# synnada-ai/datafusion-upstream

Measured on AMD Instinct MI355X. Metric: rows/sec hash-join+agg, TPC-H SF100 Q3, higher is better.
Workload: dtype int64; 1 GPU; TPC-H SF100 Q3 (3-way hash join + group-by SUM + sort), int64 keys, Decimal128(15,2) money, resident in HBM; input_rows=765043119, parallelism=1 GPU

## Files before the change

datafusion-upstream_amd/csrc/core.hip:

```cpp
#include "device_utils.h"
#include <mutex>

namespace dfgpu {

void fail(dfgpu_status code, const char* fmt, ...) {
  char buf[1024]; va_list ap; va_start(ap, fmt); vsnprintf(buf, sizeof buf, fmt, ap); va_end(ap);
  throw Error(code, buf);
}

struct CtxRefs { std::atomic<int64_t> n{1}; };
static std::mutex g_mu;
static std::vector<std::pair<dfgpu_ctx*, CtxRefs*>> g_ctx;
static CtxRefs* refs_of(dfgpu_ctx* c) { std::lock_guard<std::mutex> l(g_mu); for (auto& p : g_ctx) if (p.first == c) return p.second; return nullptr; }
static void ctx_unref(dfgpu_ctx* c) {
  CtxRefs* r = refs_of(c);
  if (!r || r->n.fetch_sub(1) != 1) return;
  { std::lock_guard<std::mutex> l(g_mu); for (size_t i = 0; i < g_ctx.size(); i++) if (g_ctx[i].first == c) { g_ctx.erase(g_ctx.begin() + i); break; } }
  (void)hipSetDevice(c->device);
  (void)hipStreamSynchronize(c->stream);
  if (c->free_blocks) { for (auto& b : *c->free_blocks) (void)hipFree(b.second); delete c->free_blocks; }
  delete c->alloc_mu;
  if (c->d_flags) (void)hipFree(c->d_flags);
  if (c->d_scratch64) (void)hipFree(c->d_scratch64);
  if (c->h_pinned) (void)hipHostFree(c->h_pinned);
// ... 294 lines not shown
  const int64_t c = counts[i];
  if (c < 0 || c > (int64_t)(0x7FFFFFF0u / w)) { atomicOr(flags, DFGPU_FLAG_OOB); lens[i] = 0; } else lens[i] = (uint32_t)c * w;
}
__global__ void __launch_bounds__(BLOCK) k_list_row_of(const int32_t* offsets, int64_t n, int64_t ne, uint32_t w, uint32_t* row_of) {
  const int64_t e = (int64_t)blockIdx.x * BLOCK + threadIdx.x; if (e >= ne) return;
  const int64_t at = (int64_t)offsets[0] + e * w;
  int64_t lo = 0, hi = n - 1;
  while (lo < hi) { const int64_t mid = (lo + hi + 1) >> 1; if ((int64_t)offsets[mid] <= at) lo = mid; else hi = mid - 1; }
  row_of[e] = (uint32_t)lo;
}
__global__ void __launch_bounds__(BLOCK) k_slist_sizes(const int32_t* voff, int64_t nv, uint32_t* enc) {
  const int64_t j = (int64_t)blockIdx.x * BLOCK + threadIdx.x; if (j > nv) return;
  enc[j] = j == nv ? 0u : 4u + (uint32_t)(voff[j + 1] - voff[j]);
}
__global__ void __launch_bounds__(BLOCK) k_slist_offsets(const uint32_t* cpre , const uint32_t* epos , int64_t n, int32_t* out_off) {
  const int64_t i = (int64_t)blockIdx.x * BLOCK + threadIdx.x; if (i <= n) out_off[i] = (int32_t)epos[cpre[i]];
}
__global__ void __launch_bounds__(BLOCK) k_slist_encode(const int32_t* voff, const uint8_t* vbytes, int64_t nv, const uint32_t* epos, uint8_t* out) {
  const int64_t j = (int64_t)blockIdx.x * BLOCK + threadIdx.x; if (j >= nv) return;
  const uint32_t len = (uint32_t)(voff[j + 1] - voff[j]); uint8_t* o = out + epos[j]; const uint8_t* src = vbytes + voff[j];
  o[0] = (uint8_t)len; o[1] = (uint8_t)(len >> 8); o[2] = (uint8_t)(len >> 16); o[3] = (uint8_t)(len >> 24);
  for (uint32_t b = 0; b < len; b++) o[4 + b] = src[b];
}
__global__ void __launch_bounds__(BLOCK) k_slist_walk(const int32_t* loff, const uint8_t* lbytes, int64_t n, const uint32_t* vstart, uint32_t* cnt, uint32_t* lens, uint32_t* spos, uint32_t* row_of, uint32_t* flags) {
  const int64_t i = (int64_t)blockIdx.x * BLOCK + threadIdx.x; if (i >= n) return;
  int64_t at = loff[i]; const int64_t end = loff[i + 1]; uint32_t k = 0;
  while (at < end) {
    if (at + 4 > end) { atomicOr(flags, DFGPU_FLAG_OOB); break; }
    const uint32_t len = (uint32_t)lbytes[at] | ((uint32_t)lbytes[at + 1] << 8) | ((uint32_t)lbytes[at + 2] << 16) | ((uint32_t)lbytes[at + 3] << 24);
    if (at + 4 + (int64_t)len > end) { atomicOr(flags, DFGPU_FLAG_OOB); break; }
    if (lens) { const uint32_t v = vstart[i] + k; lens[v] = len; spos[v] = (uint32_t)(at + 4); row_of[v] = (uint32_t)i; }
    k++; at += 4 + (int64_t)len;
  }
  if (cnt) cnt[i] = k;
}
__global__ void __launch_bounds__(BLOCK) k_slist_copy(const uint8_t* lbytes, const uint32_t* spos, const int32_t* voff, int64_t nv, uint8_t* out) {
  const int64_t j = (int64_t)blockIdx.x * BLOCK + threadIdx.x; if (j >= nv) return;
  const uint32_t len = (uint32_t)(voff[j + 1] - voff[j]); const uint8_t* src = lbytes + spos[j]; uint8_t* o = out + voff[j];
  for (uint32_t b = 0; b < len; b++) o[b] = src[b];
}

struct CtxOption { const char* name; int64_t (*get)(const dfgpu_ctx*); void (*set)(dfgpu_ctx*, int64_t); };
#define OPT_GET(M) [](const dfgpu_ctx* c) -> int64_t { return (int64_t)c->M; }
#define OPT_BOOL(M) OPT_GET(M), [](dfgpu_ctx* c, int64_t v) { c->M = v != 0; }
#define OPT_INT(M) OPT_GET(M), [](dfgpu_ctx* c, int64_t v) { c->M = v; }
#define OPT_MIN(M, LO) OPT_GET(M), [](dfgpu_ctx* c, int64_t v) { c->M = v < LO ? LO : v; }
#define OPT_RANGE(M, LO, HI) OPT_GET(M), [](dfgpu_ctx* c, int64_t v) { if (v < LO || v > HI) fail(DFGPU_INVALID_ARGUMENT, #M ": " #LO " .. " #HI); c->M = v; }
#define OPT_READ(M) OPT_GET(M), nullptr
static const CtxOption kCtxOptions[] = {
  { "force_hash_collisions", OPT_BOOL(force_hash_collisions) },
  { "first_seen_group_order", OPT_BOOL(first_seen_group_order) },
  { "join_rank_index", OPT_BOOL(join_rank_index) },
  { "join_rank_index_unsorted", OPT_BOOL(join_rank_index_unsorted) },
  { "join_lazy_build_rows", OPT_BOOL(join_lazy_build_rows) },
  { "join_selection_output", OPT_BOOL(join_selection_output) },
  { "join_probe_fused_filter", OPT_BOOL(join_probe_fused_filter) },
  { "join_key_packing", OPT_BOOL(join_key_packing) },
  { "join_swap_small_semi", OPT_BOOL(join_swap_small_semi) },
  { "join_partitioned", OPT_BOOL(join_partitioned) },
  { "join_partitioned_min_build", OPT_INT(join_partitioned_min_build) },
  { "join_partitioned_min_probe", OPT_INT(join_partitioned_min_probe) },
  { "join_partitioned_big", OPT_BOOL(join_partitioned_big) },
  { "join_partitioned_hashed", OPT_BOOL(join_partitioned_hashed) },
  { "join_partitioned_hash_mask", [](const dfgpu_ctx* c) -> int64_t { return c->join_partitioned_hash_mask == ~0ull ? 0 : (int64_t)c->join_partitioned_hash_mask; },
                                  [](dfgpu_ctx* c, int64_t v) { c->join_partitioned_hash_mask = v <= 0 ? ~0ull : (uint64_t)v; } },
  { "join_partition_rows", OPT_INT(join_partition_rows) },
  { "group_run_detection", OPT_BOOL(group_run_detection) },
  { "group_lazy_keys", OPT_BOOL(group_lazy_keys) },
  { "group_dictionary_canon", OPT_BOOL(group_dictionary_canon) },
  { "fused_aggregate_min_rows", OPT_INT(fused_aggregate_min_rows) },
  { "agg_order_inverse_map", OPT_BOOL(agg_order_inverse_map) },
  { "agg_partitioned", OPT_BOOL(agg_partitioned) },
  { "agg_partitioned_force", OPT_BOOL(agg_partitioned_force) },
  { "agg_partitioned_min_rows", OPT_INT(agg_partitioned_min_rows) },
  { "agg_pack_estimate_min_rows", OPT_INT(agg_pack_estimate_min_rows) },
  { "agg_preaggregate_distinct", OPT_READ(pa_last_distinct) },
  { "agg_spill_state_bytes", OPT_INT(agg_spill_state_bytes) },
  { "agg_spill_ranges", OPT_RANGE(agg_spill_ranges, 1, 4096) },
  { "sort_packed_keys", OPT_BOOL(sort_packed_keys) },
  { "sort_packed_min_rows", OPT_MIN(sort_packed_min_rows, 2) },
  { "sort_estimate_ranges", OPT_BOOL(sort_estimate_ranges) },
  { "sort_topk_words_min_rows", OPT_MIN(sort_topk_words_min_rows, 2) },
  { "sort_one_block_max_rows", OPT_MIN(sort_one_block_max_rows, 0) },
  { "sort_onesweep_min_rows", OPT_MIN(sort_onesweep_min_rows, 2) },
  { "sort_onesweep_rows", OPT_GET(sort_onesweep_rows), [](dfgpu_ctx* c, int64_t v) { c->sort_onesweep_rows = v == 16 ? 16 : v > 0 ? 8 : 0; } },
  { "sort_onesweep_fused_finish", OPT_BOOL(sort_onesweep_fused_finish) },
  { "sort_fused_small_passes", OPT_BOOL(sort_fused_small_passes) },
  { "sort_spill_bytes", OPT_INT(sort_spill_bytes) },
  { "sort_spill_ranges", OPT_RANGE(sort_spill_ranges, 1, 4096) },
  { "spm_merge_rows", OPT_GET(spm_merge_rows), [](dfgpu_ctx* c, int64_t v) { if (v < 0) fail(DFGPU_INVALID_ARGUMENT, "spm_merge_rows: >= 0"); c->spm_merge_rows = v; } },
  { "memory_limit", OPT_INT(memory_limit) },
  { "live_bytes", OPT_READ(live_bytes) },
  { "cached_bytes", OPT_READ(cached_bytes) },
  { "trim_cache", nullptr, [](dfgpu_ctx* c, int64_t) {
      HIP_CHECK(hipStreamSynchronize(c->stream));
      std::lock_guard<std::mutex> l(*c->alloc_mu); for (auto& x : *c->free_blocks) (void)hipFree(x.second); c->free_blocks->clear(); c->cached_bytes = 0; } },
  { "mailbox_readback", OPT_BOOL(mailbox_readback) },
  { "collect_metrics", OPT_BOOL(collect_metrics) },
  { "defer_flag_checks", OPT_GET(defer_flag_checks), [](dfgpu_ctx* c, int64_t v) {
      if (v) c->defer_flag_checks++;
      else { if (c->defer_flag_checks > 0) c->defer_flag_checks--; if (c->defer_flag_checks == 0) flush_flags(c); } } },
};
#undef OPT_GET
#undef OPT_BOOL
#undef OPT_INT
#undef OPT_MIN
// ... 406 lines not shown
```

datafusion-upstream_amd/csrc/dfgpu_internal.h:

```cpp
#pragma once
#include <hip/hip_runtime.h>
#include <atomic>
#include <cstdarg>
#include <cstdint>
#include <cstdio>
#include <cstring>
#include <memory>
#include <mutex>
#include <stdexcept>
#include <string>
#include <vector>
#include "../../include/dfgpu.h"

namespace dfgpu {

struct Error : std::exception {
  dfgpu_status code; std::string msg;
  Error(dfgpu_status c, std::string m) : code(c), msg(std::move(m)) {}
  const char* what() const noexcept override { return msg.c_str(); }
};
[[noreturn]] void fail(dfgpu_status code, const char* fmt, ...);

#define HIP_CHECK(expr)                                                                         \
  do { hipError_t e_ = (expr);                                                                  \
    if (e_ != hipSuccess) ::dfgpu::fail(e_ == hipErrorOutOfMemory ? DFGPU_RESOURCES_EXHAUSTED : DFGPU_INTERNAL, \
                                        "%s failed: %s (%s:%d)", #expr, hipGetErrorString(e_), __FILE__, __LINE__); } while (0)
#define KERNEL_CHECK() HIP_CHECK(hipGetLastError())

}

enum : uint32_t { DFGPU_FLAG_DIV_ZERO = 1, DFGPU_FLAG_OVERFLOW = 2, DFGPU_FLAG_CAST = 4, DFGPU_FLAG_OOB = 8, DFGPU_FLAG_TABLE_FULL = 16, DFGPU_FLAG_STALLED = 32 };

namespace dfgpu { struct Buffer; }
struct dfgpu_ctx {
  int device = 0;
  hipStream_t stream = nullptr;
  bool own_stream = false;
  hipStream_t copy_stream = nullptr;
  std::string err;
  bool force_hash_collisions = false;
  bool first_seen_group_order = true;
  bool join_rank_index = true;
  bool join_lazy_build_rows = true;
  bool join_selection_output = true;
  bool join_probe_fused_filter = true;
  bool join_rank_index_unsorted = true;
  bool join_key_packing = true;
  bool group_run_detection = true;
  bool group_lazy_keys = true;
  bool group_dictionary_canon = true;
  bool join_swap_small_semi = true;
  uint64_t join_partitioned_hash_mask = ~0ull;
  bool join_partitioned_hashed = true;
  bool join_partitioned_big = true;
  bool join_partitioned = true; int64_t join_partitioned_min_build = 1 << 20, join_partitioned_min_probe = 1 << 22, join_partition_rows = 14000;
  int64_t fused_aggregate_min_rows = 1 << 20;
  bool sort_packed_keys = true;
  bool agg_partitioned = true, agg_partitioned_force = false; int64_t agg_partitioned_min_rows = 1 << 22;
  bool agg_order_inverse_map = true;
  int64_t agg_pack_estimate_min_rows = 1 << 22;
  bool pa_last_distinct = false;
  const void* pa_sample_key = nullptr; const void* pa_sample_mask = nullptr; int64_t pa_sample_n = 0; uint64_t pa_sample[3] = {0, 0, 0};
  std::shared_ptr<dfgpu::Buffer> pa_pack; int pa_pack_n = 0; int64_t pa_pack_min[4] = {0, 0, 0, 0}; uint64_t pa_pack_stride[4] = {0, 0, 0, 0}, pa_pack_range[4] = {0, 0, 0, 0}; bool pa_pack_nullable[4] = {false, false, false, false};
  std::shared_ptr<dfgpu::Buffer> row_selection; int64_t row_selection_len = 0;
  int defer_flag_checks = 0; bool flags_pending = false; std::string flags_what;
  uint32_t* d_flags = nullptr;
  uint64_t* d_scratch64 = nullptr;
  uint64_t* h_pinned = nullptr;
  static constexpr int MAIL_SEQ = 384, MAIL_WORDS = 256, PINNED_WORDS = 512;
  bool mailbox_readback = true; uint64_t mail_seq = 0;
  int num_cus = 256;
  std::mutex* alloc_mu = nullptr;
  std::vector<std::pair<size_t, void*>>* free_blocks = nullptr;
  size_t cached_bytes = 0, live_bytes = 0;
  int64_t sort_packed_min_rows = 1 << 20;
  int64_t sort_topk_words_min_rows = 1 << 23;
  int64_t sort_one_block_max_rows = 8192;
  int64_t sort_onesweep_min_rows = 1 << 20;
  bool sort_onesweep_fused_finish = true;
  int sort_onesweep_rows = 16;
  bool sort_fused_small_passes = true;
  bool sort_estimate_ranges = true;
  int64_t spm_merge_rows = (int64_t)1 << 25;
  int64_t sort_spill_bytes = 0, sort_spill_ranges = 16;
  int64_t agg_spill_state_bytes = 0, agg_spill_ranges = 16;
  int64_t memory_limit = 0;
  bool collect_metrics = false;
  struct Span { hipEvent_t start = nullptr, stop = nullptr; };
  std::vector<Span> spans;
  std::mutex span_mu;
  bool profile = false; std::string profile_only;
  std::vector<std::pair<std::string, int64_t>> sync_counts;
  void count_sync(const char* why) { if (!profile) return; for (auto& kv : sync_counts) if (kv.first == why) { kv.second++; return; } sync_counts.emplace_back(why, 1); }
  struct ProfRec { const char* name; hipEvent_t start, stop; };
  std::vector<ProfRec> prof;
};

namespace dfgpu {

// ... 143 lines not shown
```

datafusion-upstream_amd/csrc/join.hip:

```cpp
#include "join_table.h"

namespace dfgpu {
constexpr uint64_t SLOT_EMPTY = ~0ull;
constexpr uint32_t NO_SLOT = 0xFFFFFFFFu;
}
using namespace dfgpu;


namespace dfgpu {

__device__ inline bool row_selected(const uint64_t* mask, int64_t i) { return mask == nullptr || bit_get(mask, i); }

__global__ void __launch_bounds__(BLOCK) k_join_build(KeySet ks, int64_t n, const uint64_t* mask, int null_eq, int force_zero,
                                                      uint64_t* slots, uint32_t* slot_count, uint64_t cap_mask, uint32_t* row_slot,
                                                      unsigned long long* counters ) {
  int64_t i = (int64_t)blockIdx.x * BLOCK + threadIdx.x;
  if (i >= n) return;
  uint32_t my_slot = NO_SLOT;
  if (row_selected(mask, i)) {
    bool any_null; uint64_t h = keyset_hash(ks, i, 0, &any_null);
    if (force_zero) h = 0;
    if (!any_null || null_eq) {
      uint64_t tag = h >> 32, s = h & cap_mask, mine = (tag << 32) | (uint64_t)i;
      for (uint64_t step = 0; step <= cap_mask; step++) {
// ... 231 lines not shown
__global__ void __launch_bounds__(BLOCK) k_key_setbits(const T* keys, const uint32_t* row_slot, int64_t n, int64_t kmin, uint64_t* bitmap) {
  int64_t i = (int64_t)blockIdx.x * BLOCK + threadIdx.x;
  if (i >= n || row_slot[i] == NO_SLOT) return;
  uint64_t d = (uint64_t)((int64_t)keys[i] - kmin);
  atomicOr((unsigned long long*)&bitmap[d >> 6], 1ull << (d & 63));
}
template <typename T>
__global__ void __launch_bounds__(BLOCK) k_check_increasing(const T* keys, int64_t n, unsigned long long* out ) {
  bool bad = false, dup = false;
  for (int64_t i = (int64_t)blockIdx.x * BLOCK + threadIdx.x + 1; i < n; i += (int64_t)gridDim.x * BLOCK) { T a = keys[i - 1], b = keys[i]; bad |= b < a; dup |= a == b; }
  if (ballot64(bad) && lane_id() == 0) out[0] = 1ull;
  if (ballot64(dup) && lane_id() == 0) out[3] = 1ull;
  if (blockIdx.x == 0 && threadIdx.x == 0) { out[1] = (unsigned long long)(long long)keys[0]; out[2] = (unsigned long long)(long long)keys[n - 1]; }
}
template <typename T>
__global__ void __launch_bounds__(BLOCK) k_key_setbits_unique(const T* keys, const uint64_t* mask, const uint32_t* rows, const unsigned long long* d_count, int64_t n, int64_t kmin, uint64_t* bitmap, unsigned long long* dup, const T* ckeys = nullptr) {
  const int64_t m = rows ? (int64_t)*d_count : n;
  for (int64_t j = (int64_t)blockIdx.x * BLOCK + threadIdx.x; j < m; j += (int64_t)gridDim.x * BLOCK) {
    const int64_t i = rows ? (int64_t)rows[j] : j;
    if (!rows && mask && !bit_get(mask, i)) continue;
    const uint64_t d = (uint64_t)((int64_t)(ckeys ? ckeys[j] : keys[i]) - kmin), bit = 1ull << (d & 63);
    const unsigned long long old = atomicOr((unsigned long long*)&bitmap[d >> 6], (unsigned long long)bit);
    if (old & bit) *dup = 1ull;
  }
}
template <typename T>
__global__ void __launch_bounds__(BLOCK) k_rank_rows(const T* keys, const uint64_t* mask, const uint32_t* rows, const unsigned long long* d_count, int64_t n, int64_t kmin, const uint64_t* bitmap, const uint32_t* prefix, uint32_t* row_of_rank, const T* ckeys = nullptr) {
  const int64_t m = rows ? (int64_t)*d_count : n;
  for (int64_t j = (int64_t)blockIdx.x * BLOCK + threadIdx.x; j < m; j += (int64_t)gridDim.x * BLOCK) {
    const int64_t i = rows ? (int64_t)rows[j] : j;
    if (!rows && mask && !bit_get(mask, i)) continue;
    const uint64_t d = (uint64_t)((int64_t)(ckeys ? ckeys[j] : keys[i]) - kmin);
    row_of_rank[prefix[d >> 6] + (uint32_t)__popcll(bitmap[d >> 6] & ((1ull << (d & 63)) - 1ull))] = (uint32_t)i;
  }
}
template <typename T>
__global__ void __launch_bounds__(BLOCK) k_key_run_heads(const T* keys, int64_t n, uint64_t* heads) {
  int64_t i = (int64_t)blockIdx.x * BLOCK + threadIdx.x;
  bool h = i < n && (i == 0 || keys[i - 1] != keys[i]);
  uint64_t m = ballot64(h);
  if (lane_id() == 0 && (i >> 6) < ((n + 63) >> 6)) heads[i >> 6] = m;
}
template <typename T>
__global__ void __launch_bounds__(BLOCK) k_probe_lookup_runs(const T* pkeys, const uint32_t* rows, int64_t m, int64_t kmin, const uint64_t* bitmap, const uint32_t* prefix,
                                                             const uint32_t* run_starts, int64_t n_runs, int64_t n_build, uint32_t* out_run, uint32_t* out_cnt) {
  int64_t i = (int64_t)blockIdx.x * BLOCK + threadIdx.x;
  if (i >= m) return;
  uint64_t d = (uint64_t)((int64_t)pkeys[rows[i]] - kmin);
  uint32_t r = prefix[d >> 6] + (uint32_t)__popcll(bitmap[d >> 6] & ((1ull << (d & 63)) - 1ull));
  uint32_t st = run_starts[r], en = (int64_t)r + 1 < n_runs ? run_starts[r + 1] : (uint32_t)n_build;
  out_run[i] = r; out_cnt[i] = en - st;
}
template <typename T>
__global__ void __launch_bounds__(BLOCK) k_key_setbits_masked(const T* keys, const uint64_t* mask, int64_t n, int64_t kmin, uint64_t* bitmap) {
  int64_t i = (int64_t)blockIdx.x * BLOCK + threadIdx.x;
  int lane = lane_id();
  bool on = i < n && row_selected(mask, i);
  uint64_t d = on ? (uint64_t)((int64_t)keys[i] - kmin) : 0;
  int64_t w = on ? (int64_t)(d >> 6) : -1 - lane;
  uint64_t b = on ? 1ull << (d & 63) : 0ull;
#pragma unroll
  for (int s = 1; s < WAVE; s <<= 1) {
    uint64_t ob = __shfl_up(b, s, 64); int64_t ow = __shfl_up(w, s, 64);
    if (lane >= s && ow == w) b |= ob;
  }
  int64_t nxt = __shfl_down(w, 1, 64);
  if (on && (lane == WAVE - 1 || nxt != w)) atomicOr((unsigned long long*)&bitmap[w], (unsigned long long)b);
}
template <typename T>
__global__ void __launch_bounds__(BLOCK) k_key_setbits_rows(const T* keys, const uint32_t* rows, const unsigned long long* d_count, int64_t kmin, uint64_t* bitmap) {
  const int64_t m = (int64_t)*d_count; const int lane = lane_id();
  for (int64_t j0 = (int64_t)blockIdx.x * BLOCK; j0 < m; j0 += (int64_t)gridDim.x * BLOCK) {
    const int64_t j = j0 + threadIdx.x; const bool on = j < m;
    uint64_t d = on ? (uint64_t)((int64_t)keys[rows[j]] - kmin) : 0;
    int64_t w = on ? (int64_t)(d >> 6) : -1 - lane;
    uint64_t b = on ? 1ull << (d & 63) : 0ull;
#pragma unroll
    for (int s2 = 1; s2 < WAVE; s2 <<= 1) {
      uint64_t ob = __shfl_up(b, s2, 64); int64_t ow = __shfl_up(w, s2, 64);
      if (lane >= s2 && ow == w) b |= ob;
    }
    int64_t nxt = __shfl_down(w, 1, 64);
    if (on && (lane == WAVE - 1 || nxt != w)) atomicOr((unsigned long long*)&bitmap[w], (unsigned long long)b);
  }
}
__global__ void __launch_bounds__(BLOCK) k_popc_words(const uint64_t* words, int64_t nw, uint32_t* out) {
  int64_t i = (int64_t)blockIdx.x * BLOCK + threadIdx.x;
  if (i < nw) out[i] = (uint32_t)__popcll(words[i]);
}
constexpr int LR_ROWS = 4;
template <typename T, bool ALL, bool SEL>
__global__ void __launch_bounds__(BLOCK) k_probe_lookup_rank(const T* pkeys, const uint32_t* rows, int64_t m, int64_t kmin, const uint64_t* bitmap,
                                                             const uint32_t* prefix, const uint32_t* sel_rows, int identity, uint64_t* out_build,
                                                             const uint64_t* rows_valid = nullptr, int64_t n_probe = 0) {
  const int64_t base = (int64_t)blockIdx.x * BLOCK * LR_ROWS + threadIdx.x;
  int64_t ic[LR_ROWS]; uint64_t d[LR_ROWS], r[LR_ROWS];
#pragma unroll
  for (int q = 0; q < LR_ROWS; q++) { int64_t i = base + (int64_t)q * BLOCK; ic[q] = i < m ? i : m - 1; }
  bool live[LR_ROWS];
#pragma unroll
  for (int q = 0; q < LR_ROWS; q++) live[q] = rows_valid == nullptr || valid_at(rows_valid, ic[q]);
  if constexpr (!ALL) {
#pragma unroll
    for (int q = 0; q < LR_ROWS; q++) ic[q] = rows[ic[q]];
  }
  if (rows_valid) {
#pragma unroll
    for (int q = 0; q < LR_ROWS; q++) if (!live[q] || ic[q] >= n_probe) ic[q] = 0;
  }
#pragma unroll
  for (int q = 0; q < LR_ROWS; q++) d[q] = live[q] ? (uint64_t)((int64_t)pkeys[ic[q]] - kmin) : 0;
  if (identity) {
#pragma unroll
    for (int q = 0; q < LR_ROWS; q++) r[q] = d[q];
  } else {
    uint64_t w[LR_ROWS]; uint32_t p[LR_ROWS];
#pragma unroll
    for (int q = 0; q < LR_ROWS; q++) { w[q] = bitmap[d[q] >> 6]; p[q] = prefix[d[q] >> 6]; }
#pragma unroll
    for (int q = 0; q < LR_ROWS; q++) r[q] = p[q] + (uint32_t)__popcll(w[q] & ((1ull << (d[q] & 63)) - 1ull));
    if constexpr (SEL) {
#pragma unroll
      for (int q = 0; q < LR_ROWS; q++) r[q] = sel_rows[r[q]];
    }
  }
#pragma unroll
  for (int q = 0; q < LR_ROWS; q++) { int64_t i = base + (int64_t)q * BLOCK; if (i < m) out_build[i] = r[q]; }
}
#define DFGPU_INT_KEY_DISPATCH(TYPE, CALL)                                                                      \
// ... 160 lines not shown
    t->csr_rows = rows;
    t->slot_start = alloc_buffer(ctx, cap * 4);
    HIP_CHECK(hipMemcpyAsync(t->slot_start->ptr, t->slot_count->ptr, cap * 4, hipMemcpyDeviceToDevice, ctx->stream));
    exclusive_scan_u32_inplace32(ctx, (uint32_t*)t->slot_start->ptr, (int64_t)cap, nullptr);
    t->mem += (int64_t)(cap * 8 + (size_t)n * 4);
  }
}

std::shared_ptr<const OrderStats> order_stats_measure(dfgpu_ctx* ctx, const dfgpu_array* a) {
  if (!a || a->type == DFGPU_DICTIONARY || !int_key_type(a->type) || a->validity || a->length < 1) return nullptr;
  const int64_t n = a->length; const void* kv = a->values->ptr;
  zero_scratch(ctx);
  DFGPU_INT_KEY_DISPATCH(a->type, hipLaunchKernelGGL((k_check_increasing<T>), dim3(grid_for(n, BLOCK * 8, ctx->num_cus * 8)), dim3(BLOCK), 0, ctx->stream, (const T*)kv, n, (unsigned long long*)ctx->d_scratch64));
  KERNEL_CHECK();
  ctx->count_sync("sync:rank_index_check"); fetch_to_pinned(ctx, 0, ctx->d_scratch64, 32);
  OrderStats st; st.sorted = ctx->h_pinned[0] == 0; st.repeats = ctx->h_pinned[3] != 0; st.exact = true; st.lo = (int64_t)ctx->h_pinned[1]; st.hi = (int64_t)ctx->h_pinned[2];
  order_stats_set(a, st);
  return order_stats_get(a);
}
static bool build_rank_index(dfgpu_ctx* ctx, dfgpu_join_table* t) {
  int64_t n = t->n_build;
  if (!ctx->join_rank_index || ctx->force_hash_collisions || n < 2 || t->nkeys != 1 || t->null_equals_null) return false;
  const dfgpu_array* key0 = t->keys[0];
  if (key0->type == DFGPU_DICTIONARY || !int_key_type(key0->type) || key0->validity) return false;
  const void* kv = key0->values->ptr;
  KernelTimer kt_(ctx, "join_build_rank");
  auto st = order_stats_get(key0);
  if (!st) st = order_stats_measure(ctx, key0);
  auto dense = [&](const OrderStats& s2) { const uint64_t r = (uint64_t)s2.hi - (uint64_t)s2.lo + 1; return r != 0 && r <= (1ull << 32) && r <= (uint64_t)n * 4096 + 65536; };
  if (st && st->sorted && !st->exact && !dense(*st)) st = order_stats_measure(ctx, key0);
  if (!st || !st->sorted) return false;
  const bool runs = st->repeats;
  if (runs && (t->build_mask || n > 0xFFFFFFF0ll)) return false;
  long long lo = (long long)st->lo, hi = (long long)st->hi;
  uint64_t range = (uint64_t)hi - (uint64_t)lo + 1;
  if (!dense(*st)) return false;
  const uint64_t* mk = t->build_mask ? (const uint64_t*)t->build_mask->ptr : nullptr;
  int64_t nw = (int64_t)((range + 63) / 64);
  t->key_min = lo; t->range = range;
  t->rep = runs ? JoinRep::RANK_RUNS : JoinRep::RANK; t->unique = !runs; t->rank_identity = !runs && range == (uint64_t)n;
  BufferPtr heads;
  if (runs) {
    heads = alloc_buffer(ctx, bitmap_bytes(n));
    DFGPU_INT_KEY_DISPATCH(key0->type, hipLaunchKernelGGL((k_key_run_heads<T>), dim3(grid_for(n, BLOCK)), dim3(BLOCK), 0, ctx->stream, (const T*)kv, n, (uint64_t*)heads->ptr));
    KERNEL_CHECK();
    mk = (const uint64_t*)heads->ptr;
  }
  if (t->rank_identity && mk) t->bitmap = t->build_mask;
  else {
    t->bitmap = alloc_buffer(ctx, bitmap_bytes((int64_t)range)); t->mem += (int64_t)bitmap_bytes((int64_t)range);
    HIP_CHECK(hipMemsetAsync(t->bitmap->ptr, t->rank_identity ? 0xFF : 0, bitmap_bytes((int64_t)range), ctx->stream));
  }
  if (!t->rank_identity) {
    if (mk && !runs && n <= 0xFFFFFFF0ll) {
      t->sel_rows = mask_to_indices_uncounted(ctx, mk, n, ctx->d_scratch64 + 15); t->mem += t->sel_rows->length * 4;
      DFGPU_INT_KEY_DISPATCH(key0->type, hipLaunchKernelGGL((k_key_setbits_rows<T>), dim3(grid_for(n, BLOCK, ctx->num_cus * 16)), dim3(BLOCK), 0, ctx->stream, (const T*)kv, (const uint32_t*)t->sel_rows->values->ptr,
                                                            (const unsigned long long*)(ctx->d_scratch64 + 15), (int64_t)lo, (uint64_t*)t->bitmap->ptr));
    } else {
      DFGPU_INT_KEY_DISPATCH(key0->type, hipLaunchKernelGGL((k_key_setbits_masked<T>), dim3(grid_for(n, BLOCK)), dim3(BLOCK), 0, ctx->stream, (const T*)kv, mk, n, (int64_t)lo, (uint64_t*)t->bitmap->ptr));
      if (mk) { t->sel_rows = mask_to_indices_impl(ctx, mk, n); t->mem += t->sel_rows->length * 4; }
    }
    KERNEL_CHECK();
    t->rank_prefix = alloc_buffer(ctx, (size_t)nw * 4);
    hipLaunchKernelGGL(k_popc_words, dim3(grid_for(nw, BLOCK)), dim3(BLOCK), 0, ctx->stream, (const uint64_t*)t->bitmap->ptr, nw, (uint32_t*)t->rank_prefix->ptr);
    exclusive_scan_u32_inplace32(ctx, (uint32_t*)t->rank_prefix->ptr, nw, nullptr);
    KERNEL_CHECK();
    t->mem += nw * 4;
  }
  return true;
}

template <typename T>
__global__ void __launch_bounds__(BLOCK) k_key_minmax_masked(const T* keys, const uint64_t* valid, const uint64_t* mask, int64_t n, long long* mn, long long* mx, const uint32_t* rows = nullptr, const unsigned long long* d_count = nullptr) {
  long long lo = INT64_MAX, hi = INT64_MIN;
  if (rows) {
    const int64_t m = (int64_t)*d_count;
    for (int64_t j = (int64_t)blockIdx.x * BLOCK + threadIdx.x; j < m; j += (int64_t)gridDim.x * BLOCK) { const int64_t i = rows[j]; if (valid_at(valid, i)) { long long v = (long long)keys[i]; lo = v < lo ? v : lo; hi = v > hi ? v : hi; } }
  } else
  for (int64_t i = (int64_t)blockIdx.x * BLOCK + threadIdx.x; i < n; i += (int64_t)gridDim.x * BLOCK)
    if (row_selected(mask, i) && valid_at(valid, i)) { long long v = (long long)keys[i]; lo = v < lo ? v : lo; hi = v > hi ? v : hi; }
#pragma unroll
  for (int d = 32; d > 0; d >>= 1) { long long a = __shfl_xor(lo, d, 64), b = __shfl_xor(hi, d, 64); lo = a < lo ? a : lo; hi = b > hi ? b : hi; }
  __shared__ long long slo[BLOCK / WAVE], shi[BLOCK / WAVE];
  if (lane_id() == 0) { slo[threadIdx.x >> 6] = lo; shi[threadIdx.x >> 6] = hi; }
  __syncthreads();
  if (threadIdx.x == 0) {
    for (int w = 1; w < BLOCK / WAVE; w++) { lo = slo[w] < lo ? slo[w] : lo; hi = shi[w] > hi ? shi[w] : hi; }
    if (lo <= hi) { atomicMin(mn, lo); atomicMax(mx, hi); }
  }
}
template <typename T>
__global__ void __launch_bounds__(BLOCK) k_key_gather_minmax(const T* keys, const uint32_t* rows, const unsigned long long* d_count, T* ckeys, long long* mn, long long* mx) {
  const int64_t m = (int64_t)*d_count; long long lo = INT64_MAX, hi = INT64_MIN;
  for (int64_t j0 = ((int64_t)blockIdx.x * BLOCK) * 4 + threadIdx.x; j0 < m; j0 += (int64_t)gridDim.x * BLOCK * 4) {
    T k[4]; bool on[4];
#pragma unroll
    for (int q = 0; q < 4; q++) { const int64_t j = j0 + (int64_t)q * BLOCK; on[q] = j < m; k[q] = on[q] ? keys[rows[j]] : (T)0; }
#pragma unroll
    for (int q = 0; q < 4; q++) if (on[q]) { ckeys[j0 + (int64_t)q * BLOCK] = k[q]; const long long v = (long long)k[q]; lo = v < lo ? v : lo; hi = v > hi ? v : hi; }
  }
#pragma unroll
  for (int d = 32; d > 0; d >>= 1) { long long a = __shfl_xor(lo, d, 64), b = __shfl_xor(hi, d, 64); lo = a < lo ? a : lo; hi = b > hi ? b : hi; }
  __shared__ long long slo[BLOCK / WAVE], shi[BLOCK / WAVE];
  if (lane_id() == 0) { slo[threadIdx.x >> 6] = lo; shi[threadIdx.x >> 6] = hi; }
  __syncthreads();
  if (threadIdx.x == 0) {
    for (int w = 1; w < BLOCK / WAVE; w++) { lo = slo[w] < lo ? slo[w] : lo; hi = shi[w] > hi ? shi[w] : hi; }
    if (lo <= hi) { atomicMin(mn, lo); atomicMax(mx, hi); }
  }
}
static bool build_rank_index_unsorted(dfgpu_ctx* ctx, dfgpu_join_table* t) {
  const int64_t n = t->n_build;
  if (!ctx->join_rank_index || !ctx->join_rank_index_unsorted || ctx->force_hash_collisions || n < 2 || n > 0xFFFFFFF0ll || t->nkeys != 1 || t->null_equals_null) return false;
  const dfgpu_array* key0 = t->keys[0];
  if (key0->type == DFGPU_DICTIONARY || !int_key_type(key0->type) || key0->validity) return false;
  KernelTimer kt_(ctx, "join_build_rank");
  const uint64_t* mk = t->build_mask ? (const uint64_t*)t->build_mask->ptr : nullptr;
  ArrayHolder list; const uint32_t* rl = nullptr; const unsigned long long* dcount = (const unsigned long long*)(ctx->d_scratch64 + 15);
  if (mk) { list.a = mask_to_indices_uncounted(ctx, mk, n, ctx->d_scratch64 + 15); rl = (const uint32_t*)list.get()->values->ptr; }
// ... 406 lines not shown
```

datafusion-upstream_amd/csrc/select.hip:

```cpp
#include "device_utils.h"
#include <algorithm>

namespace dfgpu {

struct U128 { uint64_t lo, hi; };
template <int W> struct WT;
template <> struct WT<1> { using T = uint8_t; };
template <> struct WT<2> { using T = uint16_t; };
template <> struct WT<4> { using T = uint32_t; };
template <> struct WT<8> { using T = uint64_t; };
template <> struct WT<16> { using T = U128; };

__global__ void k_iota_u32(uint32_t* out, int64_t n, uint32_t start) {
  int64_t i = (int64_t)blockIdx.x * blockDim.x + threadIdx.x;
  if (i < n) out[i] = start + (uint32_t)i;
}
void launch_iota_u32(dfgpu_ctx* ctx, uint32_t* out, int64_t n, uint32_t start) {
  if (n <= 0) return;
  hipLaunchKernelGGL(k_iota_u32, dim3(grid_for(n, BLOCK)), dim3(BLOCK), 0, ctx->stream, out, n, start);
  KERNEL_CHECK();
}

__device__ inline int64_t load_index(const void* idx, int w, int64_t i) { return w == 4 ? (int64_t)((const uint32_t*)idx)[i] : (int64_t)((const uint64_t*)idx)[i]; }

// ... 72 lines not shown
    const uint32_t orow = (uint32_t)__shfl((int)rel, lo, 64);
    const int64_t srow = (int64_t)__shfl((long long)s, lo, 64);
    if (act) out[p] = src[srow + (int64_t)(pr - orow)];
  }
}

dfgpu_array* take_impl(dfgpu_ctx* ctx, const dfgpu_array* a, const void* idx, int idx_w, const uint64_t* idx_valid, int64_t n) {
  if (n > 0xFFFFFFF0ll) fail(DFGPU_NOT_IMPLEMENTED, "take above 2^32-16 rows");
  bool need_valid = idx_valid != nullptr || a->validity != nullptr;
  int32_t vt = a->type == DFGPU_DICTIONARY ? a->key_type : a->type;
  ArrayHolder h(new_array(ctx, a->type, n, a->precision, a->scale));
  dfgpu_array* o = h.get(); o->key_type = a->key_type;
  if (need_valid) o->validity = alloc_buffer(ctx, bitmap_bytes(n), n == 0); else o->null_count = 0;
  uint64_t* ov = need_valid ? (uint64_t*)o->validity->ptr : nullptr;
  const uint64_t* sv = a->validity ? (const uint64_t*)a->validity->ptr : nullptr;
  dim3 grid(grid_for(n, BLOCK)), block(BLOCK);
  if (a->type == DFGPU_UTF8) {
    BufferPtr lens = alloc_buffer(ctx, (size_t)(n + 1) * 4), off64 = alloc_buffer(ctx, (size_t)(n + 1) * 8);
    if (n) hipLaunchKernelGGL(k_take_utf8_len, grid, block, 0, ctx->stream, (const int32_t*)a->offsets->ptr, sv, a->length, idx, idx_w, idx_valid, n, (uint32_t*)lens->ptr, ov, ctx->d_flags);
    exclusive_scan_u32(ctx, (const uint32_t*)lens->ptr, (uint64_t*)off64->ptr, n, ctx->d_scratch64 + 61);
    uint64_t total = read_scratch(ctx, 61);
    if (total > 0x7FFFFFFFull) fail(DFGPU_EXECUTION, "Arrow error: offset overflow: Utf8 output of %llu bytes exceeds i32 offsets", (unsigned long long)total);
    o->values = alloc_buffer(ctx, (size_t)total); o->values_bytes = (int64_t)total; o->offsets = alloc_buffer(ctx, (size_t)(n + 1) * 4, true);
    hipLaunchKernelGGL(k_take_utf8_copy, dim3(grid_for(n + 1, BLOCK)), block, 0, ctx->stream, (const uint8_t*)a->values->ptr, (const int32_t*)a->offsets->ptr, idx, idx_w,
                       (const uint64_t*)off64->ptr, n, (int32_t*)o->offsets->ptr, (uint8_t*)o->values->ptr, total);
    KERNEL_CHECK();
  } else if (vt == DFGPU_BOOL) {
    o->values = alloc_buffer(ctx, bitmap_bytes(n), n == 0);
    if (n) hipLaunchKernelGGL(k_take_bool, grid, block, 0, ctx->stream, (const uint64_t*)a->values->ptr, sv, a->length, idx, idx_w, idx_valid, n, (uint64_t*)o->values->ptr, ov, ctx->d_flags);
    KERNEL_CHECK();
  } else {
    int w = type_width(vt);
    o->values = alloc_buffer(ctx, (size_t)n * w);
    KernelTimer kt_(ctx, "k_take_fixed");
    if (n && !need_valid && a->length > 0 && (idx_w == 4 || idx_w == 8)) {
      dim3 pgrid(grid_for(n, BLOCK * TAKE_ROWS));
#define TAKE_PLAIN(W) case W: if (idx_w == 4) hipLaunchKernelGGL((k_take_fixed_plain<W, uint32_t>), pgrid, block, 0, ctx->stream, (const WT<W>::T*)a->values->ptr, a->length, (const uint32_t*)idx, n, (WT<W>::T*)o->values->ptr, ctx->d_flags); \
                              else hipLaunchKernelGGL((k_take_fixed_plain<W, uint64_t>), pgrid, block, 0, ctx->stream, (const WT<W>::T*)a->values->ptr, a->length, (const uint64_t*)idx, n, (WT<W>::T*)o->values->ptr, ctx->d_flags); break;
      switch (w) { TAKE_PLAIN(1) TAKE_PLAIN(2) TAKE_PLAIN(4) TAKE_PLAIN(8) TAKE_PLAIN(16) default: fail(DFGPU_INTERNAL, "take: width %d", w); }
#undef TAKE_PLAIN
    } else if (n) switch (w) {
#define TAKE_CASE(W) case W: hipLaunchKernelGGL((k_take_fixed<W>), grid, block, 0, ctx->stream, (const WT<W>::T*)a->values->ptr, sv, a->length, idx, idx_w, idx_valid, n, (WT<W>::T*)o->values->ptr, ov, ctx->d_flags); break;
      TAKE_CASE(1) TAKE_CASE(2) TAKE_CASE(4) TAKE_CASE(8) TAKE_CASE(16)
#undef TAKE_CASE
      default: fail(DFGPU_INTERNAL, "take: width %d", w);
    }
    KERNEL_CHECK();
  }
  if (a->dictionary) { o->dictionary = a->dictionary; dfgpu_array_retain(a->dictionary); }
  if (need_valid) o->null_count = -1;
  return h.release();
}

constexpr int SEL_WORDS = BLOCK;
__device__ inline uint64_t mask_word(const uint64_t* bits, int64_t w, int64_t n) {
  int64_t nw = (n + 63) >> 6; if (w >= nw) return 0;
  uint64_t x = bits[w];
  if (w == nw - 1 && (n & 63)) x &= (1ull << (n & 63)) - 1ull;
  return x;
}
__global__ void __launch_bounds__(BLOCK) k_sel_count(const uint64_t* bits, int64_t n, uint32_t* counts) {
  uint32_t c = (uint32_t)__popcll(mask_word(bits, (int64_t)blockIdx.x * SEL_WORDS + threadIdx.x, n));
  __shared__ uint32_t lds[BLOCK / WAVE];
  uint32_t tot; (void)block_exclusive_sum<uint32_t>(c, lds, &tot);
  if (threadIdx.x == 0) counts[blockIdx.x] = tot;
}
__global__ void __launch_bounds__(BLOCK) k_sel_write(const uint64_t* bits, int64_t n, const uint32_t* offsets, uint32_t* out) {
  int64_t w = (int64_t)blockIdx.x * SEL_WORDS + threadIdx.x;
  int lane = lane_id();
  uint64_t word = mask_word(bits, w, n);
  uint32_t pc = (uint32_t)__popcll(word);
  __shared__ uint32_t lds[BLOCK / WAVE];
  uint32_t tot; uint32_t ex = block_exclusive_sum<uint32_t>(pc, lds, &tot) + offsets[blockIdx.x];
  uint32_t wave_tot = wave_sum(pc);
  if (wave_tot == 0) return;
  if (wave_tot <= 8 * WAVE) {
    uint32_t row0 = (uint32_t)(w * 64);
    while (word) { out[ex++] = row0 + (uint32_t)__builtin_ctzll(word); word &= word - 1; }
  } else {
    int64_t wave_w0 = w - lane;
    for (int k = 0; k < WAVE; k++) {
      uint64_t m = __shfl(word, k, 64); uint32_t p = __shfl(ex, k, 64);
      if (m == 0) continue;
      if ((m >> lane) & 1) out[p + __popcll(m & lanemask_lt())] = (uint32_t)((wave_w0 + k) * 64 + lane);
    }
  }
}
dfgpu_array* mask_to_indices_impl(dfgpu_ctx* ctx, const uint64_t* bits, int64_t n) { return mask_to_indices_checked(ctx, bits, n, -1, nullptr); }
dfgpu_array* mask_to_indices_checked(dfgpu_ctx* ctx, const uint64_t* bits, int64_t n, int check_slot, uint64_t* check_value) {
  int64_t nw = (n + 63) / 64, nb = (nw + SEL_WORDS - 1) / SEL_WORDS;
  if (n == 0) { if (check_slot >= 0) { uint64_t v = read_scratch(ctx, check_slot); if (check_value) *check_value = v; if (v) return nullptr; } return new_fixed(ctx, DFGPU_UINT32, 0); }
  BufferPtr counts = alloc_buffer(ctx, (size_t)nb * 4);
  KernelTimer kt_(ctx, "k_sel_count+scan+write");
  hipLaunchKernelGGL(k_sel_count, dim3((unsigned)nb), dim3(BLOCK), 0, ctx->stream, bits, n, (uint32_t*)counts->ptr);
  exclusive_scan_u32_inplace32(ctx, (uint32_t*)counts->ptr, nb, ctx->d_scratch64 + 60);
  int64_t total;
  if (check_slot >= 0 && check_slot < 60) {
    const uint64_t* w = read_scratch_range(ctx, check_slot, 61 - check_slot);
    if (check_value) *check_value = w[0];
    if (w[0]) return nullptr;
    total = (int64_t)w[60 - check_slot];
  } else total = (int64_t)read_scratch(ctx, 60);
  ArrayHolder h(new_fixed(ctx, DFGPU_UINT32, total));
  if (total) hipLaunchKernelGGL(k_sel_write, dim3((unsigned)nb), dim3(BLOCK), 0, ctx->stream, bits, n, (const uint32_t*)counts->ptr, (uint32_t*)h.get()->values->ptr);
  h.get()->identity = total == n;
  { OrderStats st; st.sorted = true; st.repeats = false; st.exact = false; st.lo = 0; st.hi = n - 1; order_stats_set(h.get(), st); }
  KERNEL_CHECK();
  return h.release();
}


dfgpu_array* mask_to_indices_uncounted(dfgpu_ctx* ctx, const uint64_t* bits, int64_t n, uint64_t* d_count) {
  int64_t nw = (n + 63) / 64, nb = (nw + SEL_WORDS - 1) / SEL_WORDS;
  ArrayHolder h(new_fixed(ctx, DFGPU_UINT32, n));
  if (n == 0) { if (d_count) HIP_CHECK(hipMemsetAsync(d_count, 0, 8, ctx->stream)); return h.release(); }
  BufferPtr counts = alloc_buffer(ctx, (size_t)nb * 4);
  KernelTimer kt_(ctx, "k_sel_count+scan+write");
  hipLaunchKernelGGL(k_sel_count, dim3((unsigned)nb), dim3(BLOCK), 0, ctx->stream, bits, n, (uint32_t*)counts->ptr);
  exclusive_scan_u32_inplace32(ctx, (uint32_t*)counts->ptr, nb, d_count);
  hipLaunchKernelGGL(k_sel_write, dim3((unsigned)nb), dim3(BLOCK), 0, ctx->stream, bits, n, (const uint32_t*)counts->ptr, (uint32_t*)h.get()->values->ptr);
  KERNEL_CHECK();
  return h.release();
}

struct TakeCols { int32_t n; const void* src[8]; void* dst[8]; int32_t width[8]; };
template <typename IT>
__global__ void __launch_bounds__(BLOCK) k_take_multi_plain(TakeCols tc, const IT* idx, int64_t m, int64_t n_src, uint32_t* flags) {
  const int64_t base = (int64_t)blockIdx.x * BLOCK * TAKE_ROWS + threadIdx.x;
  int64_t j[TAKE_ROWS]; bool oob = false;
#pragma unroll
  for (int q = 0; q < TAKE_ROWS; q++) { const int64_t i = base + (int64_t)q * BLOCK; j[q] = (int64_t)idx[i < m ? i : m - 1]; const bool bad = j[q] < 0 || j[q] >= n_src; oob |= bad && i < m; if (bad) j[q] = 0; }
  for (int c = 0; c < 8; c++) {
    if (c >= tc.n) break;
#pragma unroll
    for (int q = 0; q < TAKE_ROWS; q++) {
      const int64_t i = base + (int64_t)q * BLOCK; if (i >= m) continue;
      switch (tc.width[c]) {
// ... 168 lines not shown
```

Before: 269.8 billion rows/s.

## Compute join rank prefix during bitmap build and widen mask-to-index tiles

When the build keys are sorted, the bitmap-setting kernels now also record, for each bitmap word, the first row index that lands in it. This yields the rank prefix directly and skips the separate popcount kernel and scan. Separately, the mask-to-indices select kernels now process four 64-bit words per thread using 128-bit vector loads. Each block covers more words and needs fewer partial counts. The prefix shortcut is only correct if key order is monotone and rows are dense, and it adds a memset plus extra shuffles to the build kernels.

```diff
diff --git a/datafusion-upstream_amd/csrc/core.hip b/datafusion-upstream_amd/csrc/core.hip
--- a/datafusion-upstream_amd/csrc/core.hip
+++ b/datafusion-upstream_amd/csrc/core.hip
@@ -370,6 +370,7 @@
   { "first_seen_group_order", OPT_BOOL(first_seen_group_order) },
   { "join_rank_index", OPT_BOOL(join_rank_index) },
   { "join_rank_index_unsorted", OPT_BOOL(join_rank_index_unsorted) },
+  { "join_rank_prefix_in_build", OPT_BOOL(join_rank_prefix_in_build) },
   { "join_lazy_build_rows", OPT_BOOL(join_lazy_build_rows) },
   { "join_selection_output", OPT_BOOL(join_selection_output) },
   { "join_probe_fused_filter", OPT_BOOL(join_probe_fused_filter) },
diff --git a/datafusion-upstream_amd/csrc/dfgpu_internal.h b/datafusion-upstream_amd/csrc/dfgpu_internal.h
--- a/datafusion-upstream_amd/csrc/dfgpu_internal.h
+++ b/datafusion-upstream_amd/csrc/dfgpu_internal.h
@@ -45,6 +45,7 @@
   bool join_selection_output = true;
   bool join_probe_fused_filter = true;
   bool join_rank_index_unsorted = true;
+  bool join_rank_prefix_in_build = true;
   bool join_key_packing = true;
   bool group_run_detection = true;
   bool group_lazy_keys = true;
diff --git a/datafusion-upstream_amd/csrc/join.hip b/datafusion-upstream_amd/csrc/join.hip
--- a/datafusion-upstream_amd/csrc/join.hip
+++ b/datafusion-upstream_amd/csrc/join.hip
@@ -307,13 +307,18 @@
   out_run[i] = r; out_cnt[i] = en - st;
 }
 template <typename T>
-__global__ void __launch_bounds__(BLOCK) k_key_setbits_masked(const T* keys, const uint64_t* mask, int64_t n, int64_t kmin, uint64_t* bitmap) {
+__global__ void __launch_bounds__(BLOCK) k_key_setbits_masked(const T* keys, const uint64_t* mask, int64_t n, int64_t kmin, uint64_t* bitmap, uint32_t* prefix) {
   int64_t i = (int64_t)blockIdx.x * BLOCK + threadIdx.x;
   int lane = lane_id();
   bool on = i < n && row_selected(mask, i);
   uint64_t d = on ? (uint64_t)((int64_t)keys[i] - kmin) : 0;
   int64_t w = on ? (int64_t)(d >> 6) : -1 - lane;
   uint64_t b = on ? 1ull << (d & 63) : 0ull;
+  if (prefix) {
+    int64_t prv = __shfl_up(w, 1, 64);
+    if (lane == 0) prv = on && i > 0 ? (int64_t)((uint64_t)((int64_t)keys[i - 1] - kmin) >> 6) : -1;
+    if (on && prv != w) prefix[w] = (uint32_t)i;
+  }
 #pragma unroll
   for (int s = 1; s < WAVE; s <<= 1) {
     uint64_t ob = __shfl_up(b, s, 64); int64_t ow = __shfl_up(w, s, 64);
@@ -323,13 +328,20 @@
   if (on && (lane == WAVE - 1 || nxt != w)) atomicOr((unsigned long long*)&bitmap[w], (unsigned long long)b);
 }
 template <typename T>
-__global__ void __launch_bounds__(BLOCK) k_key_setbits_rows(const T* keys, const uint32_t* rows, const unsigned long long* d_count, int64_t kmin, uint64_t* bitmap) {
+__global__ void __launch_bounds__(BLOCK) k_key_setbits_rows(const T* keys, const uint32_t* rows, const unsigned long long* d_count, int64_t kmin, uint64_t* bitmap, uint32_t* prefix) {
   const int64_t m = (int64_t)*d_count; const int lane = lane_id();
   for (int64_t j0 = (int64_t)blockIdx.x * BLOCK; j0 < m; j0 += (int64_t)gridDim.x * BLOCK) {
     const int64_t j = j0 + threadIdx.x; const bool on = j < m;
     uint64_t d = on ? (uint64_t)((int64_t)keys[rows[j]] - kmin) : 0;
     int64_t w = on ? (int64_t)(d >> 6) : -1 - lane;
     uint64_t b = on ? 1ull << (d & 63) : 0ull;
+    if (prefix) {
+      int64_t prv = -1;
+      if (lane == 0 && on && j > 0) prv = (int64_t)((uint64_t)((int64_t)keys[rows[j - 1]] - kmin) >> 6);
+      const int64_t up = __shfl_up(w, 1, 64);
+      if (lane != 0) prv = up;
+      if (on && prv != w) prefix[w] = (uint32_t)j;
+    }
 #pragma unroll
     for (int s2 = 1; s2 < WAVE; s2 <<= 1) {
       uint64_t ob = __shfl_up(b, s2, 64); int64_t ow = __shfl_up(w, s2, 64);
@@ -596,19 +608,25 @@
     HIP_CHECK(hipMemsetAsync(t->bitmap->ptr, t->rank_identity ? 0xFF : 0, bitmap_bytes((int64_t)range), ctx->stream));
   }
   if (!t->rank_identity) {
+    const bool prefix_in_build = ctx->join_rank_prefix_in_build && !runs && n <= 0xFFFFFFF0ll;
+    uint32_t* pfx = nullptr;
+    if (prefix_in_build) { t->rank_prefix = alloc_buffer(ctx, (size_t)nw * 4); pfx = (uint32_t*)t->rank_prefix->ptr; HIP_CHECK(hipMemsetAsync(pfx, 0, (size_t)nw * 4, ctx->stream)); }
     if (mk && !runs && n <= 0xFFFFFFF0ll) {
       t->sel_rows = mask_to_indices_uncounted(ctx, mk, n, ctx->d_scratch64 + 15); t->mem += t->sel_rows->length * 4;
       DFGPU_INT_KEY_DISPATCH(key0->type, hipLaunchKernelGGL((k_key_setbits_rows<T>), dim3(grid_for(n, BLOCK, ctx->num_cus * 16)), dim3(BLOCK), 0, ctx->stream, (const T*)kv, (const uint32_t*)t->sel_rows->values->ptr,
-                                                            (const unsigned long long*)(ctx->d_scratch64 + 15), (int64_t)lo, (uint64_t*)t->bitmap->ptr));
+                                                            (const unsigned long long*)(ctx->d_scratch64 + 15), (int64_t)lo, (uint64_t*)t->bitmap->ptr, pfx));
     } else {
-      DFGPU_INT_KEY_DISPATCH(key0->type, hipLaunchKernelGGL((k_key_setbits_masked<T>), dim3(grid_for(n, BLOCK)), dim3(BLOCK), 0, ctx->stream, (const T*)kv, mk, n, (int64_t)lo, (uint64_t*)t->bitmap->ptr));
+      DFGPU_INT_KEY_DISPATCH(key0->type, hipLaunchKernelGGL((k_key_setbits_masked<T>), dim3(grid_for(n, BLOCK)), dim3(BLOCK), 0, ctx->stream, (const T*)kv, mk, n, (int64_t)lo, (uint64_t*)t->bitmap->ptr, mk ? nullptr : pfx));
       if (mk) { t->sel_rows = mask_to_indices_impl(ctx, mk, n); t->mem += t->sel_rows->length * 4; }
     }
     KERNEL_CHECK();
-    t->rank_prefix = alloc_buffer(ctx, (size_t)nw * 4);
-    hipLaunchKernelGGL(k_popc_words, dim3(grid_for(nw, BLOCK)), dim3(BLOCK), 0, ctx->stream, (const uint64_t*)t->bitmap->ptr, nw, (uint32_t*)t->rank_prefix->ptr);
-    exclusive_scan_u32_inplace32(ctx, (uint32_t*)t->rank_prefix->ptr, nw, nullptr);
-    KERNEL_CHECK();
+    if (!pfx) {
+      KernelTimer kt2_(ctx, "k_popc_words+scan");
+      t->rank_prefix = alloc_buffer(ctx, (size_t)nw * 4);
+      hipLaunchKernelGGL(k_popc_words, dim3(grid_for(nw, BLOCK)), dim3(BLOCK), 0, ctx->stream, (const uint64_t*)t->bitmap->ptr, nw, (uint32_t*)t->rank_prefix->ptr);
+      exclusive_scan_u32_inplace32(ctx, (uint32_t*)t->rank_prefix->ptr, nw, nullptr);
+      KERNEL_CHECK();
+    }
     t->mem += nw * 4;
   }
   return true;
diff --git a/datafusion-upstream_amd/csrc/select.hip b/datafusion-upstream_amd/csrc/select.hip
--- a/datafusion-upstream_amd/csrc/select.hip
+++ b/datafusion-upstream_amd/csrc/select.hip
@@ -148,37 +148,61 @@
   return h.release();
 }
 
-constexpr int SEL_WORDS = BLOCK;
+constexpr int SEL_LANE_WORDS = 4;
+constexpr int SEL_WORDS = BLOCK * SEL_LANE_WORDS;
+constexpr int SEL_HALF = SEL_WORDS / 2;
 __device__ inline uint64_t mask_word(const uint64_t* bits, int64_t w, int64_t n) {
   int64_t nw = (n + 63) >> 6; if (w >= nw) return 0;
   uint64_t x = bits[w];
   if (w == nw - 1 && (n & 63)) x &= (1ull << (n & 63)) - 1ull;
   return x;
 }
+__device__ inline void sel_tile_words(const uint64_t* bits, int64_t n, uint64_t (&x)[SEL_LANE_WORDS]) {
+  const int64_t w0 = (int64_t)blockIdx.x * SEL_WORDS + 2 * (int64_t)threadIdx.x;
+  if (((uintptr_t)bits & 15) == 0 && ((int64_t)blockIdx.x + 1) * SEL_WORDS <= (n >> 6)) {
+    const ulonglong2 a = *(const ulonglong2*)(bits + w0), b = *(const ulonglong2*)(bits + w0 + SEL_HALF);
+    x[0] = a.x; x[1] = a.y; x[2] = b.x; x[3] = b.y;
+  } else {
+    x[0] = mask_word(bits, w0, n); x[1] = mask_word(bits, w0 + 1, n); x[2] = mask_word(bits, w0 + SEL_HALF, n); x[3] = mask_word(bits, w0 + SEL_HALF + 1, n);
+  }
+}
 __global__ void __launch_bounds__(BLOCK) k_sel_count(const uint64_t* bits, int64_t n, uint32_t* counts) {
-  uint32_t c = (uint32_t)__popcll(mask_word(bits, (int64_t)blockIdx.x * SEL_WORDS + threadIdx.x, n));
+  uint64_t x[SEL_LANE_WORDS]; sel_tile_words(bits, n, x);
+  uint32_t c = (uint32_t)(__popcll(x[0]) + __popcll(x[1]) + __popcll(x[2]) + __popcll(x[3]));
   __shared__ uint32_t lds[BLOCK / WAVE];
   uint32_t tot; (void)block_exclusive_sum<uint32_t>(c, lds, &tot);
   if (threadIdx.x == 0) counts[blockIdx.x] = tot;
 }
 __global__ void __launch_bounds__(BLOCK) k_sel_write(const uint64_t* bits, int64_t n, const uint32_t* offsets, uint32_t* out) {
-  int64_t w = (int64_t)blockIdx.x * SEL_WORDS + threadIdx.x;
-  int lane = lane_id();
-  uint64_t word = mask_word(bits, w, n);
-  uint32_t pc = (uint32_t)__popcll(word);
-  __shared__ uint32_t lds[BLOCK / WAVE];
-  uint32_t tot; uint32_t ex = block_exclusive_sum<uint32_t>(pc, lds, &tot) + offsets[blockIdx.x];
-  uint32_t wave_tot = wave_sum(pc);
-  if (wave_tot == 0) return;
-  if (wave_tot <= 8 * WAVE) {
-    uint32_t row0 = (uint32_t)(w * 64);
-    while (word) { out[ex++] = row0 + (uint32_t)__builtin_ctzll(word); word &= word - 1; }
-  } else {
-    int64_t wave_w0 = w - lane;
-    for (int k = 0; k < WAVE; k++) {
-      uint64_t m = __shfl(word, k, 64); uint32_t p = __shfl(ex, k, 64);
-      if (m == 0) continue;
-      if ((m >> lane) & 1) out[p + __popcll(m & lanemask_lt())] = (uint32_t)((wave_w0 + k) * 64 + lane);
+  uint64_t x[SEL_LANE_WORDS]; sel_tile_words(bits, n, x);
+  const uint32_t base = offsets[blockIdx.x];
+  const int lane = lane_id();
+  const uint32_t c[2] = { (uint32_t)(__popcll(x[0]) + __popcll(x[1])), (uint32_t)(__popcll(x[2]) + __popcll(x[3])) };
+  __shared__ uint64_t lds[BLOCK / WAVE];
+  uint64_t tot; const uint64_t ex = block_exclusive_sum<uint64_t>((uint64_t)c[0] | (uint64_t)c[1] << 32, lds, &tot);
+  if (tot == 0) return;
+  const uint32_t e[2] = { base + (uint32_t)ex, base + (uint32_t)tot + (uint32_t)(ex >> 32) };
+  const int64_t wave_w0 = (int64_t)blockIdx.x * SEL_WORDS + 2 * (int64_t)(threadIdx.x - lane);
+#pragma unroll
+  for (int q = 0; q < 2; q++) {
+    const uint32_t wave_tot = wave_sum(c[q]);
+    if (wave_tot == 0) continue;
+    uint64_t a = x[2 * q], b = x[2 * q + 1]; uint32_t p = e[q];
+    const int64_t w0 = wave_w0 + q * SEL_HALF;
+    if (wave_tot <= 16 * WAVE) {
+      uint32_t row0 = (uint32_t)((w0 + 2 * lane) * 64);
+      while (a) { out[p++] = row0 + (uint32_t)__builtin_ctzll(a); a &= a - 1; }
+      row0 += 64;
+      while (b) { out[p++] = row0 + (uint32_t)__builtin_ctzll(b); b &= b - 1; }
+    } else {
+      for (int k = 0; k < WAVE; k++) {
+        const uint64_t ma = __shfl(a, k, 64), mb = __shfl(b, k, 64); uint32_t pk = __shfl(p, k, 64);
+        if ((ma | mb) == 0) continue;
+        const uint32_t row0 = (uint32_t)((w0 + 2 * k) * 64 + lane);
+        if ((ma >> lane) & 1) out[pk + __popcll(ma & lanemask_lt())] = row0;
+        pk += (uint32_t)__popcll(ma);
+        if ((mb >> lane) & 1) out[pk + __popcll(mb & lanemask_lt())] = row0 + 64;
+      }
     }
   }
 }
```

After: 275.6 billion rows/s (median of 6 runs). 1.02x the previous value.
